# GoekeLab/m6anet

Measured on AMD Instinct MI355X. Metric: DRACH sites/sec at num_iterations=1000, higher is better.
Workload: dtype f32

## Files before the change

m6anet_amd/csrc/m6a_api.hip:

```cpp
#include "m6a_ctx.h"

#if !defined(__HIP_DEVICE_COMPILE__)
#ifndef M6A_MT_JUMP_PATH
#error "build with -DM6A_MT_JUMP_PATH=\"<repo>/m6anet_amd/assets/mt19937_jump.bin\" (m6anet_amd/build.py does)"
#endif
asm(".section .rodata\n"
    ".global m6a_mt_jump_blob\n.global m6a_mt_jump_blob_end\n.hidden m6a_mt_jump_blob\n.hidden m6a_mt_jump_blob_end\n.balign 64\n"
    "m6a_mt_jump_blob:\n.incbin \"" M6A_MT_JUMP_PATH "\"\n"
    "m6a_mt_jump_blob_end:\n.byte 0\n.previous\n");
#endif

namespace {

thread_local std::string g_create_error;

std::mutex g_live_mu;
std::vector<m6a_ctx *> g_live;
void join_background_setups()
{
    std::lock_guard<std::mutex> g(g_live_mu);
    for (m6a_ctx *c : g_live)
        if (c->warm.joinable()) c->warm.join();
    g_live.clear();
}
// ... 413 lines not shown
        hipLaunchKernelGGL(rtab_fill_kernel, dim3(gn, gx), dim3(256), 0, c->stream, b);
        HIPCHK(c, hipGetLastError());
        HIPCHK(c, hipStreamSynchronize(c->stream));
    }
    *usable = true;
    return M6A_OK;
}

int uniform_slice(m6a_ctx *c, uint32_t seed, int n, int T, int K, int jmax, const uint16_t **C)
{
    *C = nullptr;
    if (n < 2) return M6A_OK;
    std::vector<uint32_t> hist(M6A_HIST_BINS, 0u);
    hist[n] = 1;
    bool usable = false;
    int rc = ensure_rtab(c, seed, T, K, jmax, hist.data(), &usable);
    if (rc) return rc;
    if (!usable) return fail(c, M6A_ENOMEM, "no device memory for the index table of bag size %d", n);
    const int64_t slot = c->rt.slot_of_n[n], A = (int64_t)T * K;
    uint32_t total = 0;
    HIPCHK(c, hipMemcpyAsync(&total, c->rt.RS + slot * (c->rt.n_blk + 1) + c->rt.n_blk, 4, hipMemcpyDeviceToHost, c->stream));
    HIPCHK(c, hipStreamSynchronize(c->stream));
    if ((int64_t)total < A * jmax) return fail(c, M6A_ESTREAM, "MT19937 stream too short for a flush group");
    *C = c->rt.C + slot * c->rt.n_blk * 64;
    return M6A_OK;
}

int ensure_table_reg(m6a_ctx *c, uint32_t seed, int n, int T, int K, int jmax)
{
    auto &k = c->tab_reg_key;
    if (k.valid && k.seed == seed && k.n == n && k.T == T && k.K == K && k.jmax >= jmax) return M6A_OK;
    k.valid = false;
    const size_t per_j = (size_t)(T + 8) * K;
    const size_t bytes = (size_t)jmax * per_j * 2 + 4096;
    HIPCHK(c, c->tab_reg.ensure(bytes));
    HIPCHK(c, hipMemsetAsync(c->tab_reg.p, 0, bytes, c->stream));
    const uint16_t *C = nullptr;
    int rc = uniform_slice(c, seed, n, T, K, jmax, &C);
    if (rc) return rc;
    if (C) {
        const int64_t A = (int64_t)T * K;
        hipLaunchKernelGGL(rtab_to_reg_table_kernel, dim3((unsigned)((A * jmax + 255) / 256)), dim3(256), 0, c->stream,
                           C, A, (int64_t)per_j, jmax, (uint16_t *)c->tab_reg.p);
        HIPCHK(c, hipGetLastError());
    }
    k = {seed, n, T, K, jmax, true};
    return M6A_OK;
}

int ensure_table(m6a_ctx *c, uint32_t seed, int n, int T, int K, int jmax)
{
    int rc = ensure_mean_plan(c, T);
    if (rc) return rc;
    auto &k = c->tab_key;
    if (k.valid && k.seed == seed && k.n == n && k.T == T && k.K == K && k.jmax >= jmax) return M6A_OK;
    k.valid = false;
    const MeanPlan &p = c->plan;
    const int rows = (int)p.row_pass.size();
    c->iter_of.resize((size_t)rows * 64);
    for (int r = 0; r < rows; r++)
        for (int l = 0; l < 64; l++) c->iter_of[(size_t)r * 64 + l] = plan_iteration(p, r, l);
    const size_t words = (size_t)jmax * rows * 5 * 64;
    HIPCHK(c, c->tab.ensure(words * 4 + c->iter_of.size() * 4));
    int *d_iter = (int *)((uint32_t *)c->tab.p + words);
    HIPCHK(c, hipMemcpyAsync(d_iter, c->iter_of.data(), c->iter_of.size() * 4, hipMemcpyHostToDevice, c->stream));
    const uint16_t *C = nullptr;
    rc = uniform_slice(c, seed, n, T, K, jmax, &C);
    if (rc) return rc;
    if (C) {
        hipLaunchKernelGGL(rtab_to_lds_table_kernel, dim3((unsigned)((words + 255) / 256)), dim3(256), 0, c->stream,
                           C, (int64_t)T * K, K, rows, jmax, (const int *)d_iter, (uint32_t *)c->tab.p);
        HIPCHK(c, hipGetLastError());
    } else {
        HIPCHK(c, hipMemsetAsync(c->tab.p, 0, words * 4, c->stream));
    }
    k = {seed, n, T, K, jmax, true};
    return M6A_OK;
}

void prof_begin(m6a_ctx *c, int kind)
{
    Profiler &p = c->prof;
    if (!p.on || !(p.mask >> kind & 1)) return;
    if (p.used[kind] >= kMaxProfiled) { p.dropped[kind]++; return; }
    if ((int)p.start[kind].size() <= p.used[kind]) {
        hipEvent_t a, b;
        (void)hipEventCreate(&a); (void)hipEventCreate(&b);
        p.start[kind].push_back(a); p.stop[kind].push_back(b);
    }
    (void)hipEventRecord(p.start[kind][p.used[kind]], c->stream);
}
void prof_end(m6a_ctx *c, int kind)
{
    Profiler &p = c->prof;
    if (!p.on || !(p.mask >> kind & 1) || p.used[kind] >= kMaxProfiled) return;
    (void)hipEventRecord(p.stop[kind][p.used[kind]], c->stream);
    p.used[kind]++;
}

void host_bag_range(m6a_ctx *c, const int64_t *off, int64_t S);
int sync_and_check(m6a_ctx *c);

int query_bags(m6a_ctx *c, const int64_t *d_off, int64_t S)
{
    if (c->side_work) { HIPCHK(c, hipStreamSynchronize(c->s_prep)); c->side_work = false; }
    c->h_minmax[0] = ~0ull; c->h_minmax[1] = 0ull; c->h_minmax[2] = 0ull;
    HIPCHK(c, hipMemcpyAsync(c->d_minmax, c->h_minmax, 24, hipMemcpyHostToDevice, c->stream));
    HIPCHK(c, hipMemsetAsync(c->d_hist, 0, M6A_HIST_BINS * 4, c->stream));
    hipLaunchKernelGGL(bag_minmax_kernel, dim3((unsigned)std::min<int64_t>((S + 255) / 256, 512)), dim3(256), 0,
                       c->stream, d_off, S, c->d_minmax, c->d_hist);
    HIPCHK(c, hipGetLastError());
    HIPCHK(c, hipMemcpyAsync(c->h_minmax, c->d_minmax, 24, hipMemcpyDeviceToHost, c->stream));
    HIPCHK(c, hipMemcpyAsync(c->h_hist, c->d_hist, M6A_HIST_BINS * 4, hipMemcpyDeviceToHost, c->stream));
    HIPCHK(c, hipStreamSynchronize(c->stream));
    c->bag_min = (int64_t)c->h_minmax[0];
    c->bag_max = (int64_t)c->h_minmax[1];
    c->n_reads = (int64_t)c->h_minmax[2];
    return M6A_OK;
}

int bag_stats(m6a_ctx *c, const int64_t *d_off, int64_t S)
{
    const int64_t *h = c->hint_off;
    c->hint_off = nullptr;
    if (!h) return query_bags(c, d_off, S);
    if (h[0] != 0) return fail(c, M6A_EINVAL, "off[0] must be 0");
    host_bag_range(c, h, S);
    if (c->bag_min < 0) return fail(c, M6A_EINVAL, "off[] must be non-decreasing");
    unsigned long long hash = 0;
    for (int i = 0; i < M6A_HIST_BINS; i++) hash += (unsigned long long)c->h_hist[i] * m6a_bin_weight(i);
    hipStream_t st = c->s_prep ? c->s_prep : c->stream;
    if (st != c->stream) {
        HIPCHK(c, hipEventRecord(c->ev_main, c->stream));
        HIPCHK(c, hipStreamWaitEvent(st, c->ev_main, 0));
    }
    HIPCHK(c, hipMemsetAsync(c->d_minmax, 0xff, 8, st));
    HIPCHK(c, hipMemsetAsync(c->d_minmax + 1, 0, 16, st));
    HIPCHK(c, hipMemsetAsync(c->d_hist, 0, M6A_HIST_BINS * 4, st));
    hipLaunchKernelGGL(bag_minmax_kernel, dim3((unsigned)std::min<int64_t>((S + 255) / 256, 512)), dim3(256), 0,
                       st, d_off, S, c->d_minmax, c->d_hist);
    hipLaunchKernelGGL(bag_verify_kernel, dim3(1), dim3(256), 0, st, c->d_minmax, c->d_hist, (unsigned long long)c->bag_min,
                       (unsigned long long)c->bag_max, (unsigned long long)c->n_reads, hash, c->d_err);
    HIPCHK(c, hipGetLastError());
    c->side_work = true;
    return M6A_OK;
}

int launch_encode(m6a_ctx *c, const float *X, const uint8_t *km, const int64_t *off, int64_t S,
                  int64_t R, float *rp)
{
    if (R <= 0 || S <= 0) return M6A_OK;
    EncArgs a;
    a.X = X; a.site_kmers = km; a.off = off; a.wfrag = c->d_wfrag; a.emb = c->d_emb; a.read_prob = rp;
    a.wfrag2 = c->d_wfrag2; a.w1e_tab = c->d_w1e; a.bn = c->d_w1e + M6A_W1E_FLOATS; a.err = c->d_err;
    a.n_sites = S; a.n_reads = R; a.n_tiles = (R + 31) / 32; a.b3 = c->b3;
    a.clk = c->prof.clk_for(0);
#ifdef M6A_AB_W3
    const int64_t max_waves = (int64_t)c->n_cu * 12;
#else
    const int64_t max_waves = (int64_t)c->n_cu * 8;
#endif
    a.tiles_per_wave = (a.n_tiles + max_waves - 1) / max_waves;
    const int64_t waves = (a.n_tiles + a.tiles_per_wave - 1) / a.tiles_per_wave;
    const unsigned blocks = (unsigned)((waves + 3) / 4);
    const bool fits32 = S < 0x7ffffff0LL && a.n_tiles < 0x7ffffff0LL;
    if (c->enc_variant == 2 && !fits32) return fail(c, M6A_EUNSUPPORTED, "12-slot encoder: more than 2^31 sites or tiles");
// ... 17 lines not shown
    u.C = c->rt.C; u.RS = c->rt.RS; u.slot_of_n = (const int32_t *)c->ctl_dev.p + M6A_HIST_BINS;
    u.rank = (uint32_t *)c->rt_rank.p; u.order = (const uint32_t *)c->rt_order.p;
    u.c_stride = c->rt.n_blk * 64; u.n_blk = (uint32_t)c->rt.n_blk;
    u.bag_cap = (int)std::max<int64_t>(64, (nmax + 63) / 64 * 64);
    u.si_base = si_base; u.si_count = si_count;
    return u;
}

int rtab_prepare(m6a_ctx *c, PoolArgs a, int64_t nmax, int64_t gmax, uint32_t seed, bool *use)
{
    *use = false;
    const int T = a.T, K = a.K;
    const int64_t S = a.n_sites;
    const int64_t need = stream_need(gmax, T, K);
    if (nmax > M6A_RTAB_MAX_N || c->scan_driver == 1 || c->scan_driver == 2) {
        if (c->scan_driver == 3)
            return fail(c, M6A_EUNSUPPORTED, "index-table pooling needs every bag <= %d reads (largest: %lld)", M6A_RTAB_MAX_N, (long long)nmax);
        return M6A_OK;
    }
    int distinct = 0;
    const int missing = rtab_missing(c, seed, T, K, need, c->h_hist, &distinct);
    if (c->rt_credit_seed != seed || c->rt_credit_A != (int64_t)T * K) { c->rt_credit_seed = seed; c->rt_credit_A = (int64_t)T * K; c->rt_credit = 0; }
    bool use_rtab = c->scan_driver == 3 || missing == 0 || c->rt_credit + S >= (int64_t)16 * missing;
    if (use_rtab) c->rt_credit = 0; else c->rt_credit += S;
    if (!use_rtab) return M6A_OK;
    int rc = ensure_rtab(c, seed, T, K, gmax, c->h_hist, &use_rtab);
    if (rc) return rc;
    if (!use_rtab) return M6A_OK;
    a.raw = (const uint32_t *)c->raw.p; a.raw_len = c->raw_len;
    HIPCHK(c, c->rt_rank.ensure((size_t)S * 4));
    HIPCHK(c, c->rt_order.ensure((size_t)S * 4));
    HIPCHK(c, c->ctl_dev.ensure(kCtlWords * 4));
    HIPCHK(c, hipEventSynchronize(c->ev_ctl));
    uint32_t *cur = ctl_cursor(c);
    uint32_t run = 0;
    for (int n = M6A_HIST_BINS - 1; n > M6A_RTAB_SMALL_N; n--) { cur[n] = run; run += c->h_hist[n]; }
    for (int x = 0; x < 8; x++)
        for (int n = M6A_RTAB_SMALL_N - ((M6A_RTAB_SMALL_N - x) & 7); n >= 0; n -= 8) { cur[n] = run; run += c->h_hist[n]; }
    std::memcpy(ctl_slot(c), c->rt.slot_of_n, sizeof c->rt.slot_of_n);
    HIPCHK(c, hipMemcpyAsync(c->ctl_dev.p, c->h_ctl, (size_t)(M6A_HIST_BINS + M6A_RTAB_MAX_N + 1) * 4, hipMemcpyHostToDevice, c->stream));
    HIPCHK(c, hipEventRecord(c->ev_ctl, c->stream));
    const RtabUse u = rtab_use(c, nmax);
    const unsigned n_order_blocks = (unsigned)((S + 255) / 256);
    const unsigned n_chain_blocks = (unsigned)std::min<int64_t>((a.n_groups + 3) / 4, (int64_t)c->n_cu * 16);
    hipLaunchKernelGGL(rtab_prep_kernel, dim3(n_order_blocks + n_chain_blocks), dim3(256), 0, c->stream, a, u,
                       (uint32_t *)c->ctl_dev.p, (uint32_t *)c->rt_order.p, n_order_blocks);
    HIPCHK(c, hipGetLastError());
    *use = true;
    return M6A_OK;
}

int launch_pool(m6a_ctx *c, const float *rp, const int64_t *off, int64_t S, int T, int K, float thr,
                uint32_t seed, int64_t bs, int64_t spb, float *site, double *mod, bool dry)
{
    const bool prepared = c->prep.ready && c->prep.off == off && c->prep.S == S && c->prep.T == T && c->prep.K == K &&
                          c->prep.seed == seed && c->prep.bs == bs && c->prep.spb == spb;
    c->prep.ready = false;
    if (S <= 0) return M6A_OK;
    int rc = ensure_groups(c, S, bs, spb);
    if (rc) return rc;
    const int64_t nmin = c->bag_min, nmax = c->bag_max;
    if (nmin < 0 || nmax > 0x7fffffff) return fail(c, M6A_EINVAL, "off[] is not a non-decreasing CSR array");

    PoolArgs a;
    memset(&a, 0, sizeof a);
    a.read_prob = rp; a.off = off; a.goff = (const int64_t *)c->goff.p; a.site_prob = site; a.mod_ratio = mod;
    a.err = c->d_err; a.n_groups = c->goff_key.G; a.n_sites = S; a.T = T; a.K = K; a.thr = thr;
    a.clk = dry ? nullptr : c->prof.clk_for(1);
    const int64_t gmax = c->goff_key.gmax;

    rc = ensure_mean_plan(c, T);
    if (rc) return rc;
    const bool uniform = nmin == nmax && nmin >= 1 && nmin <= M6A_TABLE_MAX_N && K == 20 && gmax <= 4096;
    const bool reg_ok = uniform && c->plan.depth <= M6A_REG_STACK && c->n_reads < (int64_t)1 << 30 &&
                        (int64_t)gmax * (T + 8) * K * 2 <= (int64_t)256 << 20;
    if (uniform && reg_ok && c->table_variant != 1) {
        rc = ensure_table_reg(c, seed, (int)nmin, T, K, (int)gmax);
        if (rc) return rc;
        plan_args(c, a);
        a.tab = (const uint32_t *)c->tab_reg.p; a.uniform_n = (int)nmin; a.jmax = (int)gmax;
        if (dry) return M6A_OK;
        c->pool_variant = "table-reg";
        prof_begin(c, 1);
        const int64_t wpj = (a.n_groups + 255) / 256;
        a.reg_items = wpj * a.jmax;
        hipLaunchKernelGGL(pool_reg_kernel, dim3((unsigned)((a.reg_items + 7) / 8 * 8)), dim3(64), 0, c->stream, a);
        prof_end(c, 1);
    } else if (uniform && c->plan.max_merge <= 15) {
        rc = ensure_table(c, seed, (int)nmin, T, K, (int)gmax);
        if (rc) return rc;
        if (dry) return M6A_OK;
        plan_args(c, a);
        a.tab = (const uint32_t *)c->tab.p; a.uniform_n = (int)nmin; a.jmax = (int)gmax;
        const int64_t gblocks = (a.n_groups + 7) / 8;
        int64_t nbj = std::max<int64_t>(1, ((int64_t)c->n_cu * 5 + a.jmax - 1) / a.jmax);
        nbj = std::min<int64_t>(nbj, (gblocks + 3) / 4);
        const unsigned blocks = (unsigned)(nbj * a.jmax);
        c->pool_variant = "table";
        prof_begin(c, 1);
        const size_t mean_lds = (size_t)4 * (128 + 8 * a.stack_depth) * sizeof(float);
        hipLaunchKernelGGL(pool_table_kernel, dim3(blocks), dim3(256), mean_lds, c->stream, a);
        prof_end(c, 1);
    } else {
        const int64_t need = stream_need(gmax, T, K);
        bool use_rtab = false;
        if (prepared && !dry) {
            use_rtab = c->prep.use;
        } else {
            rc = rtab_prepare(c, a, nmax, gmax, seed, &use_rtab);
            if (rc) return rc;
        }
        if (dry) {
            c->prep.ready = true; c->prep.use = use_rtab;
            c->prep.off = off; c->prep.S = S; c->prep.bs = bs; c->prep.spb = spb; c->prep.T = T; c->prep.K = K; c->prep.seed = seed;
            if (!use_rtab) {
                rc = ensure_raw(c, seed, need);
                if (rc) return rc;
                HIPCHK(c, c->start_pos.ensure((size_t)S * sizeof(uint32_t)));
            }
            return M6A_OK;
        }
        if (use_rtab) {
            plan_args(c, a);
            a.raw = (const uint32_t *)c->raw.p; a.raw_len = c->raw_len;
            c->pool_variant = "ragged-table";
            int64_t n_big = 0;
            for (int n = M6A_RTAB_SMALL_N + 1; n < M6A_HIST_BINS; n++) n_big += c->h_hist[n];
            prof_begin(c, 1);
            auto launch = [&](int64_t base, int64_t count, int64_t cap_n) {
                if (count <= 0) return;
                const RtabUse u = rtab_use(c, cap_n, (uint32_t)base, (uint32_t)count);
                const size_t lds = (size_t)(u.bag_cap + 16 + M6A_MEAN_STACK) * sizeof(float);
                const unsigned blocks = (unsigned)((count + 7) / 8 * 8);
                if (K == 20) hipLaunchKernelGGL(pool_rtab_kernel<20>, dim3(blocks), dim3(64), lds, c->stream, a, u);
                else hipLaunchKernelGGL(pool_rtab_kernel<0>, dim3(blocks), dim3(64), lds, c->stream, a, u);
            };
            launch(0, n_big, nmax);
            launch(n_big, S - n_big, std::min<int64_t>(nmax, M6A_RTAB_SMALL_N));
            prof_end(c, 1);
            HIPCHK(c, hipGetLastError());
            return M6A_OK;
        }
        rc = ensure_raw(c, seed, need);
        if (rc) return rc;
        plan_args(c, a);
        a.raw = (const uint32_t *)c->raw.p; a.raw_len = c->raw_len;
        HIPCHK(c, c->start_pos.ensure((size_t)S * sizeof(uint32_t)));
        a.start_pos = (uint32_t *)c->start_pos.p;
        int64_t cap = 64;
        while (cap < nmax && cap < M6A_BAG_LDS) cap *= 2;
        a.bag_cap = (int)cap;
        const size_t lds = (size_t)4 * (a.bag_cap + (32 * K + 256) * 5 / 4 + 32 + M6A_MEAN_STACK) * sizeof(float);
        const int64_t wg_per_cu = std::max<int64_t>(1, std::min<int64_t>(a.bag_cap >= 256 ? 5 : 8, (160 * 1024) / (int64_t)lds));
        const int64_t wave_slots = (int64_t)c->n_cu * wg_per_cu * 4;
        const bool by_group = c->scan_driver ? c->scan_driver == 1 : a.n_groups * 5 >= wave_slots * 3;
        c->pool_variant = by_group ? "scan-group" : "scan-site";
        prof_begin(c, 1);
        if (by_group) {
            const unsigned blocks = (unsigned)std::min<int64_t>((a.n_groups + 3) / 4, wave_slots / 4);
            if (K == 20) hipLaunchKernelGGL(pool_scan_group_kernel<20>, dim3(blocks), dim3(256), lds, c->stream, a);
            else hipLaunchKernelGGL(pool_scan_group_kernel<0>, dim3(blocks), dim3(256), lds, c->stream, a);
        } else {
            hipLaunchKernelGGL(pool_scan_start_kernel, dim3((unsigned)std::min<int64_t>((a.n_groups + 3) / 4, (int64_t)c->n_cu * 8)),
                               dim3(256), 0, c->stream, a);
            const unsigned blocks = (unsigned)std::min<int64_t>((S + 3) / 4, wave_slots / 4);
            if (K == 20) hipLaunchKernelGGL(pool_scan_site_kernel<20>, dim3(blocks), dim3(256), lds, c->stream, a);
            else hipLaunchKernelGGL(pool_scan_site_kernel<0>, dim3(blocks), dim3(256), lds, c->stream, a);
// ... 651 lines not shown
```

m6anet_amd/csrc/m6a_pool_reg.hip:

```cpp
#include "m6a_kernels.h"

#define S1(x) #x
#define S(x) S1(x)

#define MUL0 \
    "v_pk_mul_f32 v[56:57], v[128:129], 1.0 op_sel_hi:[1,0]\n" \
    "v_pk_mul_f32 v[58:59], v[192:193], 1.0 op_sel_hi:[1,0]\n"
#define MUL \
    "v_pk_mul_f32 v[56:57], v[128:129], v[56:57]\n" \
    "v_pk_mul_f32 v[58:59], v[192:193], v[58:59]\n"
#define LO(r) "s_sext_i32_i16 m0, s[" S(r) "]\n"
#define HI(r) "s_lshr_b32 m0, s[" S(r) "], 16\n"
#define DRAW2(r) LO(r) MUL HI(r) MUL
#define DRAWS(b) \
    "s_set_gpr_idx_on s[" S(b) "], gpr_idx(SRC0)\n" \
    MUL0 HI(b) MUL \
    DRAW2(b+1) DRAW2(b+2) DRAW2(b+3) DRAW2(b+4) DRAW2(b+5) DRAW2(b+6) DRAW2(b+7) DRAW2(b+8) DRAW2(b+9) \
    "s_set_gpr_idx_off\n" \
    "v_pk_add_f32 v[56:57], v[56:57], 1.0 op_sel_hi:[1,0] neg_lo:[1,0] neg_hi:[1,0]\n" \
    "v_pk_add_f32 v[58:59], v[58:59], 1.0 op_sel_hi:[1,0] neg_lo:[1,0] neg_hi:[1,0]\n"

#define ITER(i, b) \
    DRAWS(b) \
    "v_pk_add_f32 v[96+4*" S(i) ":97+4*" S(i) "], v[96+4*" S(i) ":97+4*" S(i) "], v[56:57]\n" \
    "v_pk_add_f32 v[98+4*" S(i) ":99+4*" S(i) "], v[98+4*" S(i) ":99+4*" S(i) "], v[58:59]\n"

#define COMBINE \
    "v_pk_add_f32 v[60:61], v[96:97], v[100:101]\n" \
    "v_pk_add_f32 v[40:41], v[104:105], v[108:109]\n" \
    "v_pk_add_f32 v[62:63], v[98:99], v[102:103]\n" \
    "v_pk_add_f32 v[42:43], v[106:107], v[110:111]\n" \
    "v_pk_add_f32 v[60:61], v[60:61], v[40:41]\n" \
    "v_pk_add_f32 v[62:63], v[62:63], v[42:43]\n" \
    "v_pk_add_f32 v[40:41], v[112:113], v[116:117]\n" \
    "v_pk_add_f32 v[44:45], v[120:121], v[124:125]\n" \
    "v_pk_add_f32 v[42:43], v[114:115], v[118:119]\n" \
    "v_pk_add_f32 v[46:47], v[122:123], v[126:127]\n" \
    "v_pk_add_f32 v[40:41], v[40:41], v[44:45]\n" \
    "v_pk_add_f32 v[42:43], v[42:43], v[46:47]\n" \
    "v_pk_add_f32 v[60:61], v[60:61], v[40:41]\n" \
    "v_pk_add_f32 v[62:63], v[62:63], v[42:43]\n" \
    ".set m6a_i, 0\n" \
    ".rept 32\n" \
    "v_mov_b32 v[96+m6a_i], 0\n" \
    ".set m6a_i, m6a_i+1\n" \
    ".endr\n"

#define MERGES(lbl) \
    "s_cmp_eq_u32 s79, 0\n" \
    "s_cbranch_scc1 " lbl "f\n" \
    lbl "0:\n" \
    "s_sub_u32 s78, s78, 4\n" \
    "s_set_gpr_idx_on s78, gpr_idx(SRC0)\n" \
    "v_pk_add_f32 v[60:61], v[64:65], v[60:61]\n" \
    "v_pk_add_f32 v[62:63], v[66:67], v[62:63]\n" \
    "s_set_gpr_idx_off\n" \
    "s_sub_u32 s79, s79, 1\n" \
    "s_cmp_lg_u32 s79, 0\n" \
    "s_cbranch_scc1 " lbl "0b\n" \
    lbl ":\n"

__global__ __launch_bounds__(64) void pool_reg_kernel(PoolArgs a)
{
    const int lane = threadIdx.x;
    const unsigned per = gridDim.x >> 3;
    const unsigned item = (blockIdx.x & 7u) * per + (blockIdx.x >> 3);
    if (item >= (unsigned)a.reg_items) return;
    m6a_clk_stamp(a.clk, 0);
    const int j = (int)(item % (unsigned)a.jmax);
    const int64_t g0 = (int64_t)(item / (unsigned)a.jmax) * 256;
    int64_t site[4];
    uint32_t boff[4];
#pragma unroll
    for (int q = 0; q < 4; q++) {
        const int64_t g = g0 + q * 64 + lane;
        site[q] = -1;
        if (g < a.n_groups) {
            const int64_t s = a.goff[g] + j;
            if (s < a.goff[g + 1]) site[q] = s;
        }
        boff[q] = site[q] >= 0 ? (uint32_t)(a.off[site[q]] * 4) : 0u;
    }
    const uint64_t rp = (uint64_t)a.read_prob;
    const uint64_t tab = (uint64_t)((const uint8_t *)a.tab + (size_t)j * (size_t)(a.T + 8) * 40);
    const uint64_t ctl = (uint64_t)a.reg_ctl;
    float o0, o1, o2, o3;
    int c0, c1, c2, c3;
    asm volatile(
        "v_mov_b32 v32, %[b0]\n"
        "v_mov_b32 v33, %[b1]\n"
        "v_mov_b32 v34, %[b2]\n"
        "v_mov_b32 v35, %[b3]\n"
        "s_mov_b64 s[80:81], %[tab]\n"
        "s_mov_b64 s[82:83], %[ctl]\n"
        "s_load_dwordx16 s[36:51], s[80:81], 0\n"
        "s_load_dwordx4 s[52:55], s[80:81], 64\n"
        "s_load_dwordx16 s[56:71], s[80:81], 80\n"
        "s_load_dwordx4 s[72:75], s[80:81], 144\n"
        "s_mov_b32 s77, %[nr]\n"
        "s_mov_b32 s78, 0\n"
        "v_mov_b32 v40, 0\n"
        "v_mov_b32 v41, 0\n"
        "v_mov_b32 v42, 0\n"
        "v_mov_b32 v43, 0\n"
        "s_and_b32 s79, %[n], 3\n"
        "s_cmp_eq_u32 s79, 0\n"
        "s_cbranch_scc0 80f\n"
        "s_lshr_b32 s79, %[n], 2\n"
        ".set m6a_e, 0\n"
        ".rept 8\n"
        "s_cmp_lt_u32 m6a_e, s79\n"
        "s_cbranch_scc0 81f\n"
        "global_load_dwordx4 v[64+4*m6a_e:67+4*m6a_e], v32, %[rp] offset:16*m6a_e\n"
        "global_load_dwordx4 v[96+4*m6a_e:99+4*m6a_e], v33, %[rp] offset:16*m6a_e\n"
        "global_load_dwordx4 v[128+4*m6a_e:131+4*m6a_e], v34, %[rp] offset:16*m6a_e\n"
        "global_load_dwordx4 v[160+4*m6a_e:163+4*m6a_e], v35, %[rp] offset:16*m6a_e\n"
        ".set m6a_e, m6a_e+1\n"
        ".endr\n"
        "81:\n"
        "s_waitcnt vmcnt(0)\n"
        ".set m6a_e, 0\n"
        ".rept 32\n"
        "s_cmp_lt_u32 m6a_e, %[n]\n"
        "s_cselect_b64 s[84:85], exec, 0\n"
        "v_cmp_le_f32 vcc, %[thr], v[64+m6a_e]\n"
        "s_and_b64 vcc, vcc, s[84:85]\n"
        "v_addc_co_u32 v40, vcc, 0, v40, vcc\n"
        "v_cmp_le_f32 vcc, %[thr], v[96+m6a_e]\n"
        "s_and_b64 vcc, vcc, s[84:85]\n"
        "v_addc_co_u32 v41, vcc, 0, v41, vcc\n"
        "v_cmp_le_f32 vcc, %[thr], v[128+m6a_e]\n"
        "s_and_b64 vcc, vcc, s[84:85]\n"
        "v_addc_co_u32 v42, vcc, 0, v42, vcc\n"
        "v_cmp_le_f32 vcc, %[thr], v[160+m6a_e]\n"
        "s_and_b64 vcc, vcc, s[84:85]\n"
        "v_addc_co_u32 v43, vcc, 0, v43, vcc\n"
        ".set m6a_e, m6a_e+1\n"
        ".endr\n"
        ".set m6a_e, 0\n"
        ".rept 32\n"
        "v_sub_f32 v[192+2*m6a_e], 1.0, v[128+m6a_e]\n"
        "v_sub_f32 v[193+2*m6a_e], 1.0, v[160+m6a_e]\n"
        ".set m6a_e, m6a_e+1\n"
        ".endr\n"
        ".set m6a_e, 0\n"
        ".rept 32\n"
        "v_sub_f32 v[128+2*m6a_e], 1.0, v[64+m6a_e]\n"
        "v_sub_f32 v[129+2*m6a_e], 1.0, v[96+m6a_e]\n"
        ".set m6a_e, m6a_e+1\n"
        ".endr\n"
        ".set m6a_i, 0\n"
        ".rept 64\n"
        "v_mov_b32 v[64+m6a_i], 0\n"
        ".set m6a_i, m6a_i+1\n"
        ".endr\n"
        "s_branch 82f\n"
        "80:\n"
        "s_sub_u32 s79, %[n], 1\n"
        ".set m6a_e, 0\n"
        ".rept 32\n"
        "global_load_dword v[128+2*m6a_e], v32, %[rp]\n"
        "s_cmp_lt_u32 m6a_e, s79\n"
        "s_cselect_b32 s76, 4, 0\n"
        "v_add_u32 v32, s76, v32\n"
        ".set m6a_e, m6a_e+1\n"
        ".endr\n"
        ".set m6a_e, 0\n"
        ".rept 32\n"
        "global_load_dword v[129+2*m6a_e], v33, %[rp]\n"
        "s_cmp_lt_u32 m6a_e, s79\n"
        "s_cselect_b32 s76, 4, 0\n"
        "v_add_u32 v33, s76, v33\n"
        ".set m6a_e, m6a_e+1\n"
        ".endr\n"
        ".set m6a_e, 0\n"
        ".rept 32\n"
        "global_load_dword v[192+2*m6a_e], v34, %[rp]\n"
        "s_cmp_lt_u32 m6a_e, s79\n"
        "s_cselect_b32 s76, 4, 0\n"
        "v_add_u32 v34, s76, v34\n"
        ".set m6a_e, m6a_e+1\n"
        ".endr\n"
        ".set m6a_e, 0\n"
        ".rept 32\n"
        "global_load_dword v[193+2*m6a_e], v35, %[rp]\n"
        "s_cmp_lt_u32 m6a_e, s79\n"
        "s_cselect_b32 s76, 4, 0\n"
        "v_add_u32 v35, s76, v35\n"
        ".set m6a_e, m6a_e+1\n"
        ".endr\n"
        ".set m6a_i, 0\n"
        ".rept 64\n"
        "v_mov_b32 v[64+m6a_i], 0\n"
        ".set m6a_i, m6a_i+1\n"
        ".endr\n"
        "s_waitcnt vmcnt(0)\n"
        ".set m6a_e, 0\n"
        ".rept 32\n"
        "s_cmp_lt_u32 m6a_e, %[n]\n"
        "s_cselect_b64 s[84:85], exec, 0\n"
        "v_cmp_le_f32 vcc, %[thr], v[128+2*m6a_e]\n"
        "s_and_b64 vcc, vcc, s[84:85]\n"
        "v_addc_co_u32 v40, vcc, 0, v40, vcc\n"
        "v_cmp_le_f32 vcc, %[thr], v[129+2*m6a_e]\n"
        "s_and_b64 vcc, vcc, s[84:85]\n"
        "v_addc_co_u32 v41, vcc, 0, v41, vcc\n"
        "v_cmp_le_f32 vcc, %[thr], v[192+2*m6a_e]\n"
        "s_and_b64 vcc, vcc, s[84:85]\n"
        "v_addc_co_u32 v42, vcc, 0, v42, vcc\n"
        "v_cmp_le_f32 vcc, %[thr], v[193+2*m6a_e]\n"
        "s_and_b64 vcc, vcc, s[84:85]\n"
        "v_addc_co_u32 v43, vcc, 0, v43, vcc\n"
        ".set m6a_e, m6a_e+1\n"
        ".endr\n"
        ".set m6a_i, 0\n"
        ".rept 128\n"
        "v_sub_f32 v[128+m6a_i], 1.0, v[128+m6a_i]\n"
        ".set m6a_i, m6a_i+1\n"
        ".endr\n"
        "82:\n"
        "v_mov_b32 %[c0], v40\n"
        "v_mov_b32 %[c1], v41\n"
        "v_mov_b32 %[c2], v42\n"
        "v_mov_b32 %[c3], v43\n"
        "s_waitcnt lgkmcnt(0)\n"
        "s_cmp_eq_u32 s77, 0\n"
        "s_cbranch_scc1 3f\n"
        "1:\n"
        "s_load_dword s76, s[82:83], 0\n"
        ITER(0, 36) ITER(1, 46)
        "s_waitcnt lgkmcnt(0)\n"
        "s_load_dwordx16 s[36:51], s[80:81], 160\n"
        "s_load_dwordx4 s[52:55], s[80:81], 224\n"
        ITER(2, 56) ITER(3, 66)
        "s_waitcnt lgkmcnt(0)\n"
        "s_load_dwordx16 s[56:71], s[80:81], 240\n"
        "s_load_dwordx4 s[72:75], s[80:81], 304\n"
        ITER(4, 36) ITER(5, 46)
        "s_waitcnt lgkmcnt(0)\n"
        "s_load_dwordx16 s[36:51], s[80:81], 320\n"
        "s_load_dwordx4 s[52:55], s[80:81], 384\n"
        ITER(6, 56) ITER(7, 66)
        "s_waitcnt lgkmcnt(0)\n"
        "s_load_dwordx16 s[56:71], s[80:81], 400\n"
        "s_load_dwordx4 s[72:75], s[80:81], 464\n"
        "s_add_u32 s80, s80, 320\n"
        "s_addc_u32 s81, s81, 0\n"
        "s_add_u32 s82, s82, 4\n"
        "s_addc_u32 s83, s83, 0\n"
        "s_bitcmp1_b32 s76, 0\n"
        "s_cbranch_scc0 2f\n"
        COMBINE
        "s_lshr_b32 s79, s76, 8\n"
        MERGES("4")
        "s_set_gpr_idx_on s78, gpr_idx(DST)\n"
        "v_mov_b32 v64, v60\n"
        "v_mov_b32 v65, v61\n"
        "v_mov_b32 v66, v62\n"
        "v_mov_b32 v67, v63\n"
        "s_set_gpr_idx_off\n"
        "s_add_u32 s78, s78, 4\n"
        "2:\n"
        "s_sub_u32 s77, s77, 1\n"
        "s_cmp_lg_u32 s77, 0\n"
        "s_cbranch_scc1 1b\n"
        "3:\n"
        "s_waitcnt lgkmcnt(0)\n"
        COMBINE
        "s_mov_b32 s77, %[nt]\n"
        "s_cmp_eq_u32 s77, 0\n"
        "s_cbranch_scc1 6f\n"
        "5:\n"
        "s_load_dwordx8 s[36:43], s[80:81], 0\n"
        "s_load_dwordx2 s[44:45], s[80:81], 32\n"
        "s_waitcnt lgkmcnt(0)\n"
        DRAWS(36)
        "v_pk_add_f32 v[60:61], v[60:61], v[56:57]\n"
        "v_pk_add_f32 v[62:63], v[62:63], v[58:59]\n"
        "s_add_u32 s80, s80, 40\n"
        "s_addc_u32 s81, s81, 0\n"
        "s_sub_u32 s77, s77, 1\n"
        "s_cmp_lg_u32 s77, 0\n"
        "s_cbranch_scc1 5b\n"
        "6:\n"
        "s_mov_b32 s79, %[fm]\n"
        MERGES("7")
        "v_mov_b32 %[o0], v60\n"
        "v_mov_b32 %[o1], v61\n"
        "v_mov_b32 %[o2], v62\n"
        "v_mov_b32 %[o3], v63\n"
        : [o0] "=v"(o0), [o1] "=v"(o1), [o2] "=v"(o2), [o3] "=v"(o3), [c0] "=&v"(c0), [c1] "=&v"(c1), [c2] "=&v"(c2), [c3] "=&v"(c3)
        : [thr] "s"(a.thr), [b0] "v"(boff[0]), [b1] "v"(boff[1]), [b2] "v"(boff[2]), [b3] "v"(boff[3]), [rp] "s"(rp), [tab] "s"(tab),
          [ctl] "s"(ctl), [n] "s"(a.uniform_n), [nr] "s"(a.reg_rounds), [nt] "s"(a.n_rem), [fm] "s"(a.reg_final_merges)
        : "memory", "scc", "vcc",
          "s36", "s37", "s38", "s39", "s40", "s41", "s42", "s43", "s44", "s45", "s46", "s47", "s48", "s49", "s50", "s51",
          "s52", "s53", "s54", "s55", "s56", "s57", "s58", "s59", "s60", "s61", "s62", "s63", "s64", "s65", "s66", "s67",
          "s68", "s69", "s70", "s71", "s72", "s73", "s74", "s75", "s76", "s77", "s78", "s79", "s80", "s81", "s82", "s83", "s84", "s85",
          "v32", "v33", "v34", "v35", "v40", "v41", "v42", "v43", "v44", "v45", "v46", "v47", "v56", "v57", "v58", "v59",
          "v60", "v61", "v62", "v63", "v64", "v65", "v66", "v67", "v68", "v69", "v70", "v71", "v72", "v73", "v74", "v75",
          "v76", "v77", "v78", "v79", "v80", "v81", "v82", "v83", "v84", "v85", "v86", "v87", "v88", "v89", "v90", "v91",
          "v92", "v93", "v94", "v95", "v96", "v97", "v98", "v99", "v100", "v101", "v102", "v103", "v104", "v105", "v106",
          "v107", "v108", "v109", "v110", "v111", "v112", "v113", "v114", "v115", "v116", "v117", "v118", "v119", "v120",
          "v121", "v122", "v123", "v124", "v125", "v126", "v127", "v128", "v129", "v130", "v131", "v132", "v133", "v134",
          "v135", "v136", "v137", "v138", "v139", "v140", "v141", "v142", "v143", "v144", "v145", "v146", "v147", "v148",
          "v149", "v150", "v151", "v152", "v153", "v154", "v155", "v156", "v157", "v158", "v159", "v160", "v161", "v162",
          "v163", "v164", "v165", "v166", "v167", "v168", "v169", "v170", "v171", "v172", "v173", "v174", "v175", "v176",
          "v177", "v178", "v179", "v180", "v181", "v182", "v183", "v184", "v185", "v186", "v187", "v188", "v189", "v190",
          "v191", "v192", "v193", "v194", "v195", "v196", "v197", "v198", "v199", "v200", "v201", "v202", "v203", "v204",
          "v205", "v206", "v207", "v208", "v209", "v210", "v211", "v212", "v213", "v214", "v215", "v216", "v217", "v218",
          "v219", "v220", "v221", "v222", "v223", "v224", "v225", "v226", "v227", "v228", "v229", "v230", "v231", "v232",
          "v233", "v234", "v235", "v236", "v237", "v238", "v239", "v240", "v241", "v242", "v243", "v244", "v245", "v246",
          "v247", "v248", "v249", "v250", "v251", "v252", "v253", "v254", "v255");
    const float o[4] = {o0, o1, o2, o3};
    const int cge[4] = {c0, c1, c2, c3};
#pragma unroll
    for (int q = 0; q < 4; q++) {
        if (site[q] >= 0) {
            a.site_prob[site[q]] = o[q] / (float)a.T;
            a.mod_ratio[site[q]] = (double)cge[q] / (double)a.uniform_n;
        }
    }
    m6a_clk_stamp(a.clk, 1);
}

__global__ void m6a_touch_pool_reg() {}
```

Baseline: 387.9 million.

## Halve per-wave group count in register pool kernel to cut VGPR usage

The register-resident pool kernel now handles two 64-lane groups of sites per wave instead of four. Every VGPR bank in the inline assembly is remapped into v20–v127, so the kernel needs about half as many registers. The host launch doubles the number of work items to match. The intent is higher occupancy, so more waves can hide the latency of the table draws and global loads, at the cost of more waves each reloading the same scalar table data. A profiler change also clears the clock-stamp buffer before each profiled launch.

```diff
diff --git a/m6anet_amd/csrc/m6a_api.hip b/m6anet_amd/csrc/m6a_api.hip
--- a/m6anet_amd/csrc/m6a_api.hip
+++ b/m6anet_amd/csrc/m6a_api.hip
@@ -519,6 +519,7 @@
 {
     Profiler &p = c->prof;
     if (!p.on || !(p.mask >> kind & 1)) return;
+    if (p.d_clk) (void)hipMemsetAsync(p.d_clk + (size_t)kind * M6A_CLK_SLOTS * 4, 0, (size_t)M6A_CLK_SLOTS * 4 * sizeof(unsigned long long), c->stream);
     if (p.used[kind] >= kMaxProfiled) { p.dropped[kind]++; return; }
     if ((int)p.start[kind].size() <= p.used[kind]) {
         hipEvent_t a, b;
@@ -702,7 +703,7 @@
         if (dry) return M6A_OK;
         c->pool_variant = "table-reg";
         prof_begin(c, 1);
-        const int64_t wpj = (a.n_groups + 255) / 256;
+        const int64_t wpj = (a.n_groups + 127) / 128;
         a.reg_items = wpj * a.jmax;
         hipLaunchKernelGGL(pool_reg_kernel, dim3((unsigned)((a.reg_items + 7) / 8 * 8)), dim3(64), 0, c->stream, a);
         prof_end(c, 1);
diff --git a/m6anet_amd/csrc/m6a_pool_reg.hip b/m6anet_amd/csrc/m6a_pool_reg.hip
--- a/m6anet_amd/csrc/m6a_pool_reg.hip
+++ b/m6anet_amd/csrc/m6a_pool_reg.hip
@@ -3,12 +3,8 @@
 #define S1(x) #x
 #define S(x) S1(x)
 
-#define MUL0 \
-    "v_pk_mul_f32 v[56:57], v[128:129], 1.0 op_sel_hi:[1,0]\n" \
-    "v_pk_mul_f32 v[58:59], v[192:193], 1.0 op_sel_hi:[1,0]\n"
-#define MUL \
-    "v_pk_mul_f32 v[56:57], v[128:129], v[56:57]\n" \
-    "v_pk_mul_f32 v[58:59], v[192:193], v[58:59]\n"
+#define MUL0 "v_pk_mul_f32 v[28:29], v[64:65], 1.0 op_sel_hi:[1,0]\n"
+#define MUL "v_pk_mul_f32 v[28:29], v[64:65], v[28:29]\n"
 #define LO(r) "s_sext_i32_i16 m0, s[" S(r) "]\n"
 #define HI(r) "s_lshr_b32 m0, s[" S(r) "], 16\n"
 #define DRAW2(r) LO(r) MUL HI(r) MUL
@@ -17,32 +13,23 @@
     MUL0 HI(b) MUL \
     DRAW2(b+1) DRAW2(b+2) DRAW2(b+3) DRAW2(b+4) DRAW2(b+5) DRAW2(b+6) DRAW2(b+7) DRAW2(b+8) DRAW2(b+9) \
     "s_set_gpr_idx_off\n" \
-    "v_pk_add_f32 v[56:57], v[56:57], 1.0 op_sel_hi:[1,0] neg_lo:[1,0] neg_hi:[1,0]\n" \
-    "v_pk_add_f32 v[58:59], v[58:59], 1.0 op_sel_hi:[1,0] neg_lo:[1,0] neg_hi:[1,0]\n"
+    "v_pk_add_f32 v[28:29], v[28:29], 1.0 op_sel_hi:[1,0] neg_lo:[1,0] neg_hi:[1,0]\n"
 
 #define ITER(i, b) \
     DRAWS(b) \
-    "v_pk_add_f32 v[96+4*" S(i) ":97+4*" S(i) "], v[96+4*" S(i) ":97+4*" S(i) "], v[56:57]\n" \
-    "v_pk_add_f32 v[98+4*" S(i) ":99+4*" S(i) "], v[98+4*" S(i) ":99+4*" S(i) "], v[58:59]\n"
+    "v_pk_add_f32 v[48+2*" S(i) ":49+2*" S(i) "], v[48+2*" S(i) ":49+2*" S(i) "], v[28:29]\n"
 
 #define COMBINE \
-    "v_pk_add_f32 v[60:61], v[96:97], v[100:101]\n" \
-    "v_pk_add_f32 v[40:41], v[104:105], v[108:109]\n" \
-    "v_pk_add_f32 v[62:63], v[98:99], v[102:103]\n" \
-    "v_pk_add_f32 v[42:43], v[106:107], v[110:111]\n" \
-    "v_pk_add_f32 v[60:61], v[60:61], v[40:41]\n" \
-    "v_pk_add_f32 v[62:63], v[62:63], v[42:43]\n" \
-    "v_pk_add_f32 v[40:41], v[112:113], v[116:117]\n" \
-    "v_pk_add_f32 v[44:45], v[120:121], v[124:125]\n" \
-    "v_pk_add_f32 v[42:43], v[114:115], v[118:119]\n" \
-    "v_pk_add_f32 v[46:47], v[122:123], v[126:127]\n" \
-    "v_pk_add_f32 v[40:41], v[40:41], v[44:45]\n" \
-    "v_pk_add_f32 v[42:43], v[42:43], v[46:47]\n" \
-    "v_pk_add_f32 v[60:61], v[60:61], v[40:41]\n" \
-    "v_pk_add_f32 v[62:63], v[62:63], v[42:43]\n" \
+    "v_pk_add_f32 v[30:31], v[48:49], v[50:51]\n" \
+    "v_pk_add_f32 v[20:21], v[52:53], v[54:55]\n" \
+    "v_pk_add_f32 v[30:31], v[30:31], v[20:21]\n" \
+    "v_pk_add_f32 v[20:21], v[56:57], v[58:59]\n" \
+    "v_pk_add_f32 v[22:23], v[60:61], v[62:63]\n" \
+    "v_pk_add_f32 v[20:21], v[20:21], v[22:23]\n" \
+    "v_pk_add_f32 v[30:31], v[30:31], v[20:21]\n" \
     ".set m6a_i, 0\n" \
-    ".rept 32\n" \
-    "v_mov_b32 v[96+m6a_i], 0\n" \
+    ".rept 16\n" \
+    "v_mov_b32 v[48+m6a_i], 0\n" \
     ".set m6a_i, m6a_i+1\n" \
     ".endr\n"
 
@@ -50,10 +37,9 @@
     "s_cmp_eq_u32 s79, 0\n" \
     "s_cbranch_scc1 " lbl "f\n" \
     lbl "0:\n" \
-    "s_sub_u32 s78, s78, 4\n" \
+    "s_sub_u32 s78, s78, 2\n" \
     "s_set_gpr_idx_on s78, gpr_idx(SRC0)\n" \
-    "v_pk_add_f32 v[60:61], v[64:65], v[60:61]\n" \
-    "v_pk_add_f32 v[62:63], v[66:67], v[62:63]\n" \
+    "v_pk_add_f32 v[30:31], v[32:33], v[30:31]\n" \
     "s_set_gpr_idx_off\n" \
     "s_sub_u32 s79, s79, 1\n" \
     "s_cmp_lg_u32 s79, 0\n" \
@@ -68,29 +54,27 @@
     if (item >= (unsigned)a.reg_items) return;
     m6a_clk_stamp(a.clk, 0);
     const int j = (int)(item % (unsigned)a.jmax);
-    const int64_t g0 = (int64_t)(item / (unsigned)a.jmax) * 256;
-    int64_t site[4];
-    uint32_t boff[4];
+    const int64_t g0 = (int64_t)(item / (unsigned)a.jmax) * 128;
+    int64_t site[2];
+    uint32_t boff[2];
 #pragma unroll
-    for (int q = 0; q < 4; q++) {
-        const int64_t g = g0 + q * 64 + lane;
-        site[q] = -1;
+    for (int k = 0; k < 2; k++) {
+        const int64_t g = g0 + k * 64 + lane;
+        site[k] = -1;
         if (g < a.n_groups) {
             const int64_t s = a.goff[g] + j;
-            if (s < a.goff[g + 1]) site[q] = s;
+            if (s < a.goff[g + 1]) site[k] = s;
         }
-        boff[q] = site[q] >= 0 ? (uint32_t)(a.off[site[q]] * 4) : 0u;
+        boff[k] = site[k] >= 0 ? (uint32_t)(a.off[site[k]] * 4) : 0u;
     }
     const uint64_t rp = (uint64_t)a.read_prob;
     const uint64_t tab = (uint64_t)((const uint8_t *)a.tab + (size_t)j * (size_t)(a.T + 8) * 40);
     const uint64_t ctl = (uint64_t)a.reg_ctl;
-    float o0, o1, o2, o3;
-    int c0, c1, c2, c3;
+    float o0, o1;
+    int c0, c1;
     asm volatile(
-        "v_mov_b32 v32, %[b0]\n"
-        "v_mov_b32 v33, %[b1]\n"
-        "v_mov_b32 v34, %[b2]\n"
-        "v_mov_b32 v35, %[b3]\n"
+        "v_mov_b32 v24, %[b0]\n"
+        "v_mov_b32 v25, %[b1]\n"
         "s_mov_b64 s[80:81], %[tab]\n"
         "s_mov_b64 s[82:83], %[ctl]\n"
         "s_load_dwordx16 s[36:51], s[80:81], 0\n"
@@ -99,10 +83,8 @@
         "s_load_dwordx4 s[72:75], s[80:81], 144\n"
         "s_mov_b32 s77, %[nr]\n"
         "s_mov_b32 s78, 0\n"
-        "v_mov_b32 v40, 0\n"
-        "v_mov_b32 v41, 0\n"
-        "v_mov_b32 v42, 0\n"
-        "v_mov_b32 v43, 0\n"
+        "v_mov_b32 v26, 0\n"
+        "v_mov_b32 v27, 0\n"
         "s_and_b32 s79, %[n], 3\n"
         "s_cmp_eq_u32 s79, 0\n"
         "s_cbranch_scc0 80f\n"
@@ -111,10 +93,8 @@
         ".rept 8\n"
         "s_cmp_lt_u32 m6a_e, s79\n"
         "s_cbranch_scc0 81f\n"
-        "global_load_dwordx4 v[64+4*m6a_e:67+4*m6a_e], v32, %[rp] offset:16*m6a_e\n"
-        "global_load_dwordx4 v[96+4*m6a_e:99+4*m6a_e], v33, %[rp] offset:16*m6a_e\n"
-        "global_load_dwordx4 v[128+4*m6a_e:131+4*m6a_e], v34, %[rp] offset:16*m6a_e\n"
-        "global_load_dwordx4 v[160+4*m6a_e:163+4*m6a_e], v35, %[rp] offset:16*m6a_e\n"
+        "global_load_dwordx4 v[96+4*m6a_e:99+4*m6a_e], v24, %[rp] offset:16*m6a_e\n"
+        "global_load_dwordx4 v[32+4*m6a_e:35+4*m6a_e], v25, %[rp] offset:16*m6a_e\n"
         ".set m6a_e, m6a_e+1\n"
         ".endr\n"
         "81:\n"
@@ -123,35 +103,23 @@
         ".rept 32\n"
         "s_cmp_lt_u32 m6a_e, %[n]\n"
         "s_cselect_b64 s[84:85], exec, 0\n"
-        "v_cmp_le_f32 vcc, %[thr], v[64+m6a_e]\n"
-        "s_and_b64 vcc, vcc, s[84:85]\n"
-        "v_addc_co_u32 v40, vcc, 0, v40, vcc\n"
         "v_cmp_le_f32 vcc, %[thr], v[96+m6a_e]\n"
         "s_and_b64 vcc, vcc, s[84:85]\n"
-        "v_addc_co_u32 v41, vcc, 0, v41, vcc\n"
-        "v_cmp_le_f32 vcc, %[thr], v[128+m6a_e]\n"
-        "s_and_b64 vcc, vcc, s[84:85]\n"
-        "v_addc_co_u32 v42, vcc, 0, v42, vcc\n"
-        "v_cmp_le_f32 vcc, %[thr], v[160+m6a_e]\n"
-        "s_and_b64 vcc, vcc, s[84:85]\n"
-        "v_addc_co_u32 v43, vcc, 0, v43, vcc\n"
-        ".set m6a_e, m6a_e+1\n"
-        ".endr\n"
-        ".set m6a_e, 0\n"
-        ".rept 32\n"
-        "v_sub_f32 v[192+2*m6a_e], 1.0, v[128+m6a_e]\n"
-        "v_sub_f32 v[193+2*m6a_e], 1.0, v[160+m6a_e]\n"
-        ".set m6a_e, m6a_e+1\n"
-        ".endr\n"
-        ".set m6a_e, 0\n"
-        ".rept 32\n"
-        "v_sub_f32 v[128+2*m6a_e], 1.0, v[64+m6a_e]\n"
-        "v_sub_f32 v[129+2*m6a_e], 1.0, v[96+m6a_e]\n"
+        "v_addc_co_u32 v26, vcc, 0, v26, vcc\n"
+        "v_cmp_le_f32 vcc, %[thr], v[32+m6a_e]\n"
+        "s_and_b64 vcc, vcc, s[84:85]\n"
+        "v_addc_co_u32 v27, vcc, 0, v27, vcc\n"
+        ".set m6a_e, m6a_e+1\n"
+        ".endr\n"
+        ".set m6a_e, 0\n"
+        ".rept 32\n"
+        "v_sub_f32 v[64+2*m6a_e], 1.0, v[96+m6a_e]\n"
+        "v_sub_f32 v[65+2*m6a_e], 1.0, v[32+m6a_e]\n"
         ".set m6a_e, m6a_e+1\n"
         ".endr\n"
         ".set m6a_i, 0\n"
-        ".rept 64\n"
-        "v_mov_b32 v[64+m6a_i], 0\n"
+        ".rept 32\n"
+        "v_mov_b32 v[32+m6a_i], 0\n"
         ".set m6a_i, m6a_i+1\n"
         ".endr\n"
         "s_branch 82f\n"
@@ -159,70 +127,46 @@
         "s_sub_u32 s79, %[n], 1\n"
         ".set m6a_e, 0\n"
         ".rept 32\n"
-        "global_load_dword v[128+2*m6a_e], v32, %[rp]\n"
+        "global_load_dword v[64+2*m6a_e], v24, %[rp]\n"
         "s_cmp_lt_u32 m6a_e, s79\n"
         "s_cselect_b32 s76, 4, 0\n"
-        "v_add_u32 v32, s76, v32\n"
-        ".set m6a_e, m6a_e+1\n"
-        ".endr\n"
-        ".set m6a_e, 0\n"
-        ".rept 32\n"
-        "global_load_dword v[129+2*m6a_e], v33, %[rp]\n"
+        "v_add_u32 v24, s76, v24\n"
+        ".set m6a_e, m6a_e+1\n"
+        ".endr\n"
+        ".set m6a_e, 0\n"
+        ".rept 32\n"
+        "global_load_dword v[65+2*m6a_e], v25, %[rp]\n"
         "s_cmp_lt_u32 m6a_e, s79\n"
         "s_cselect_b32 s76, 4, 0\n"
-        "v_add_u32 v33, s76, v33\n"
-        ".set m6a_e, m6a_e+1\n"
-        ".endr\n"
-        ".set m6a_e, 0\n"
-        ".rept 32\n"
-        "global_load_dword v[192+2*m6a_e], v34, %[rp]\n"
-        "s_cmp_lt_u32 m6a_e, s79\n"
-        "s_cselect_b32 s76, 4, 0\n"
-        "v_add_u32 v34, s76, v34\n"
-        ".set m6a_e, m6a_e+1\n"
-        ".endr\n"
-        ".set m6a_e, 0\n"
-        ".rept 32\n"
-        "global_load_dword v[193+2*m6a_e], v35, %[rp]\n"
-        "s_cmp_lt_u32 m6a_e, s79\n"
-        "s_cselect_b32 s76, 4, 0\n"
-        "v_add_u32 v35, s76, v35\n"
+        "v_add_u32 v25, s76, v25\n"
+        ".set m6a_e, m6a_e+1\n"
+        ".endr\n"
+        ".set m6a_i, 0\n"
+        ".rept 32\n"
+        "v_mov_b32 v[32+m6a_i], 0\n"
+        ".set m6a_i, m6a_i+1\n"
+        ".endr\n"
+        "s_waitcnt vmcnt(0)\n"
+        ".set m6a_e, 0\n"
+        ".rept 32\n"
+        "s_cmp_lt_u32 m6a_e, %[n]\n"
+        "s_cselect_b64 s[84:85], exec, 0\n"
+        "v_cmp_le_f32 vcc, %[thr], v[64+2*m6a_e]\n"
+        "s_and_b64 vcc, vcc, s[84:85]\n"
+        "v_addc_co_u32 v26, vcc, 0, v26, vcc\n"
+        "v_cmp_le_f32 vcc, %[thr], v[65+2*m6a_e]\n"
+        "s_and_b64 vcc, vcc, s[84:85]\n"
+        "v_addc_co_u32 v27, vcc, 0, v27, vcc\n"
         ".set m6a_e, m6a_e+1\n"
         ".endr\n"
         ".set m6a_i, 0\n"
         ".rept 64\n"
-        "v_mov_b32 v[64+m6a_i], 0\n"
+        "v_sub_f32 v[64+m6a_i], 1.0, v[64+m6a_i]\n"
         ".set m6a_i, m6a_i+1\n"
         ".endr\n"
-        "s_waitcnt vmcnt(0)\n"
-        ".set m6a_e, 0\n"
-        ".rept 32\n"
-        "s_cmp_lt_u32 m6a_e, %[n]\n"
-        "s_cselect_b64 s[84:85], exec, 0\n"
-        "v_cmp_le_f32 vcc, %[thr], v[128+2*m6a_e]\n"
-        "s_and_b64 vcc, vcc, s[84:85]\n"
-        "v_addc_co_u32 v40, vcc, 0, v40, vcc\n"
-        "v_cmp_le_f32 vcc, %[thr], v[129+2*m6a_e]\n"
-        "s_and_b64 vcc, vcc, s[84:85]\n"
-        "v_addc_co_u32 v41, vcc, 0, v41, vcc\n"
-        "v_cmp_le_f32 vcc, %[thr], v[192+2*m6a_e]\n"
-        "s_and_b64 vcc, vcc, s[84:85]\n"
-        "v_addc_co_u32 v42, vcc, 0, v42, vcc\n"
-        "v_cmp_le_f32 vcc, %[thr], v[193+2*m6a_e]\n"
-        "s_and_b64 vcc, vcc, s[84:85]\n"
-        "v_addc_co_u32 v43, vcc, 0, v43, vcc\n"
-        ".set m6a_e, m6a_e+1\n"
-        ".endr\n"
-        ".set m6a_i, 0\n"
-        ".rept 128\n"
-        "v_sub_f32 v[128+m6a_i], 1.0, v[128+m6a_i]\n"
-        ".set m6a_i, m6a_i+1\n"
-        ".endr\n"
         "82:\n"
-        "v_mov_b32 %[c0], v40\n"
-        "v_mov_b32 %[c1], v41\n"
-        "v_mov_b32 %[c2], v42\n"
-        "v_mov_b32 %[c3], v43\n"
+        "v_mov_b32 %[c0], v26\n"
+        "v_mov_b32 %[c1], v27\n"
         "s_waitcnt lgkmcnt(0)\n"
         "s_cmp_eq_u32 s77, 0\n"
         "s_cbranch_scc1 3f\n"
@@ -254,12 +198,10 @@
         "s_lshr_b32 s79, s76, 8\n"
         MERGES("4")
         "s_set_gpr_idx_on s78, gpr_idx(DST)\n"
-        "v_mov_b32 v64, v60\n"
-        "v_mov_b32 v65, v61\n"
-        "v_mov_b32 v66, v62\n"
-        "v_mov_b32 v67, v63\n"
+        "v_mov_b32 v32, v30\n"
+        "v_mov_b32 v33, v31\n"
         "s_set_gpr_idx_off\n"
-        "s_add_u32 s78, s78, 4\n"
+        "s_add_u32 s78, s78, 2\n"
         "2:\n"
         "s_sub_u32 s77, s77, 1\n"
         "s_cmp_lg_u32 s77, 0\n"
@@ -275,8 +217,7 @@
         "s_load_dwordx2 s[44:45], s[80:81], 32\n"
         "s_waitcnt lgkmcnt(0)\n"
         DRAWS(36)
-        "v_pk_add_f32 v[60:61], v[60:61], v[56:57]\n"
-        "v_pk_add_f32 v[62:63], v[62:63], v[58:59]\n"
+        "v_pk_add_f32 v[30:31], v[30:31], v[28:29]\n"
         "s_add_u32 s80, s80, 40\n"
         "s_addc_u32 s81, s81, 0\n"
         "s_sub_u32 s77, s77, 1\n"
@@ -285,39 +226,30 @@
         "6:\n"
         "s_mov_b32 s79, %[fm]\n"
         MERGES("7")
-        "v_mov_b32 %[o0], v60\n"
-        "v_mov_b32 %[o1], v61\n"
-        "v_mov_b32 %[o2], v62\n"
-        "v_mov_b32 %[o3], v63\n"
-        : [o0] "=v"(o0), [o1] "=v"(o1), [o2] "=v"(o2), [o3] "=v"(o3), [c0] "=&v"(c0), [c1] "=&v"(c1), [c2] "=&v"(c2), [c3] "=&v"(c3)
-        : [thr] "s"(a.thr), [b0] "v"(boff[0]), [b1] "v"(boff[1]), [b2] "v"(boff[2]), [b3] "v"(boff[3]), [rp] "s"(rp), [tab] "s"(tab),
+        "v_mov_b32 %[o0], v30\n"
+        "v_mov_b32 %[o1], v31\n"
+        : [o0] "=v"(o0), [o1] "=v"(o1), [c0] "=&v"(c0), [c1] "=&v"(c1)
+        : [thr] "s"(a.thr), [b0] "v"(boff[0]), [b1] "v"(boff[1]), [rp] "s"(rp), [tab] "s"(tab),
           [ctl] "s"(ctl), [n] "s"(a.uniform_n), [nr] "s"(a.reg_rounds), [nt] "s"(a.n_rem), [fm] "s"(a.reg_final_merges)
         : "memory", "scc", "vcc",
           "s36", "s37", "s38", "s39", "s40", "s41", "s42", "s43", "s44", "s45", "s46", "s47", "s48", "s49", "s50", "s51",
           "s52", "s53", "s54", "s55", "s56", "s57", "s58", "s59", "s60", "s61", "s62", "s63", "s64", "s65", "s66", "s67",
           "s68", "s69", "s70", "s71", "s72", "s73", "s74", "s75", "s76", "s77", "s78", "s79", "s80", "s81", "s82", "s83", "s84", "s85",
-          "v32", "v33", "v34", "v35", "v40", "v41", "v42", "v43", "v44", "v45", "v46", "v47", "v56", "v57", "v58", "v59",
-          "v60", "v61", "v62", "v63", "v64", "v65", "v66", "v67", "v68", "v69", "v70", "v71", "v72", "v73", "v74", "v75",
-          "v76", "v77", "v78", "v79", "v80", "v81", "v82", "v83", "v84", "v85", "v86", "v87", "v88", "v89", "v90", "v91",
-          "v92", "v93", "v94", "v95", "v96", "v97", "v98", "v99", "v100", "v101", "v102", "v103", "v104", "v105", "v106",
-          "v107", "v108", "v109", "v110", "v111", "v112", "v113", "v114", "v115", "v116", "v117", "v118", "v119", "v120",
-          "v121", "v122", "v123", "v124", "v125", "v126", "v127", "v128", "v129", "v130", "v131", "v132", "v133", "v134",
-          "v135", "v136", "v137", "v138", "v139", "v140", "v141", "v142", "v143", "v144", "v145", "v146", "v147", "v148",
-          "v149", "v150", "v151", "v152", "v153", "v154", "v155", "v156", "v157", "v158", "v159", "v160", "v161", "v162",
-          "v163", "v164", "v165", "v166", "v167", "v168", "v169", "v170", "v171", "v172", "v173", "v174", "v175", "v176",
-          "v177", "v178", "v179", "v180", "v181", "v182", "v183", "v184", "v185", "v186", "v187", "v188", "v189", "v190",
-          "v191", "v192", "v193", "v194", "v195", "v196", "v197", "v198", "v199", "v200", "v201", "v202", "v203", "v204",
-          "v205", "v206", "v207", "v208", "v209", "v210", "v211", "v212", "v213", "v214", "v215", "v216", "v217", "v218",
-          "v219", "v220", "v221", "v222", "v223", "v224", "v225", "v226", "v227", "v228", "v229", "v230", "v231", "v232",
-          "v233", "v234", "v235", "v236", "v237", "v238", "v239", "v240", "v241", "v242", "v243", "v244", "v245", "v246",
-          "v247", "v248", "v249", "v250", "v251", "v252", "v253", "v254", "v255");
-    const float o[4] = {o0, o1, o2, o3};
-    const int cge[4] = {c0, c1, c2, c3};
+          "v20", "v21", "v22", "v23", "v24", "v25", "v26", "v27", "v28", "v29", "v30", "v31", "v32", "v33", "v34",
+          "v35", "v36", "v37", "v38", "v39", "v40", "v41", "v42", "v43", "v44", "v45", "v46", "v47", "v48", "v49",
+          "v50", "v51", "v52", "v53", "v54", "v55", "v56", "v57", "v58", "v59", "v60", "v61", "v62", "v63", "v64",
+          "v65", "v66", "v67", "v68", "v69", "v70", "v71", "v72", "v73", "v74", "v75", "v76", "v77", "v78", "v79",
+          "v80", "v81", "v82", "v83", "v84", "v85", "v86", "v87", "v88", "v89", "v90", "v91", "v92", "v93", "v94",
+          "v95", "v96", "v97", "v98", "v99", "v100", "v101", "v102", "v103", "v104", "v105", "v106", "v107", "v108",
+          "v109", "v110", "v111", "v112", "v113", "v114", "v115", "v116", "v117", "v118", "v119", "v120", "v121",
+          "v122", "v123", "v124", "v125", "v126", "v127");
+    const float o[2] = {o0, o1};
+    const int cge[2] = {c0, c1};
 #pragma unroll
-    for (int q = 0; q < 4; q++) {
-        if (site[q] >= 0) {
-            a.site_prob[site[q]] = o[q] / (float)a.T;
-            a.mod_ratio[site[q]] = (double)cge[q] / (double)a.uniform_n;
+    for (int k = 0; k < 2; k++) {
+        if (site[k] >= 0) {
+            a.site_prob[site[k]] = o[k] / (float)a.T;
+            a.mod_ratio[site[k]] = (double)cge[k] / (double)a.uniform_n;
         }
     }
     m6a_clk_stamp(a.clk, 1);
```

After: 388.8 million (median of 6 runs). About the same (+0.2%).
